# FudanCVL/SynFMC

Hardware: AMD Instinct MI355X
Metric: denoising steps/sec, 16x320x512 bf16 U-Net+CMC+OMC (higher is better)
Workload: dtype bf16; 1 GPU; 16x320x512 clip, CFG batch 2, full-width 3D U-Net (1.39B params, random init) + Camera Adapter (CMC) + Object Motion Control (OMC) features, DDIM step; configs/obj.yaml shapes; 1 clip per GPU; frames=16, height=320, width=512, hip_graph=True, fp8_temporal_attention=False, parallelism=dp1 (independent clips, no collective)

## Files before the change

include/fmc_hip.h:

```cpp
#ifndef FMC_HIP_H
#define FMC_HIP_H

#include <stdint.h>

#ifdef __cplusplus
extern "C" {
#endif

#define FMC_VERSION 100

enum { FMC_BF16 = 0, FMC_F32 = 1 };

enum {
    FMC_OK = 0,
    FMC_E_SHAPE = -1,
    FMC_E_DTYPE = -2,
    FMC_E_ALIGN = -3,
    FMC_E_LAUNCH = -4,
    FMC_E_NULL = -5
};

int fmc_version(void);
const char* fmc_last_error(void);

// ... 179 lines not shown
    int N, K;
    float alpha;
    int accumulate;
} fmc_wgrad_problem;
int64_t fmc_linear_wgrad_workspace_bytes(const fmc_wgrad_problem* problems, int n_problems);
int fmc_linear_wgrad_bf16(const fmc_wgrad_problem* problems, int n_problems, void* workspace, int64_t workspace_bytes, void* stream);

int fmc_temporal_block_bf16(const void* h, void* out, const float* ln_gamma, const float* ln_bpe, float ln_eps, const void* w_merge_tm,
                            const void* pose_term, float merge_scale, const void* w_qkv_packed, const void* w_out_tm, const void* b_out,
                            float* ln_stats, float ln_stats_eps, int n_clips, int frames, int hw, int channels, int heads, float scale,
                            void* stream);
int fmc_xattn_block640_bf16(const void* h, void* out, const float* ln_gamma, const float* ln_bpe, float ln_eps, const void* w_q_packed,
                            const void* kvfrag, const void* w_out_frag, const void* b_out, int n_images, int hw, int n_keys, int images_per_text,
                            float scale, void* stream);
int fmc_xattn_pack_kv(const void* kv, void* out, int batch, int S, int64_t ld_batch, void* stream);
int fmc_xattn_block320_bf16(const void* h, void* out, const float* ln_gamma, const float* ln_bpe, float ln_eps, const void* w_q_packed,
                            const void* kvfrag, const void* w_out_tm, const void* b_out, float* ln_stats, float ln_stats_eps, int n_images, int hw,
                            int n_keys, int images_per_text, float scale, void* stream);
int fmc_xattn_pack_kv40(const void* kv, void* out, int batch, int S, int64_t ld_batch, void* stream);
int fmc_geglu640_ln_bf16(const void* h, void* out, const float* ln_gamma, const float* ln_beta, float ln_eps, const void* w_packed, const void* bias,
                         int64_t M, int cff, int out_blocked, void* stream);
int fmc_geglu320_ln_bf16(const void* h, void* out, const float* ln_gamma, const float* ln_beta, float ln_eps, const void* w_packed, const void* bias,
                         int64_t M, int cff, int out_blocked, void* stream);
int fmc_temporal_block_set_debug(void* buf);

enum { FMC_OPTIM_ZERO_GRAD = 1 };
typedef struct fmc_optim_tensor {
    float* p;
    float* g;
    float* m;
    float* v;
    uint16_t* shadow_bf16;
    float* shadow_f32;
    float* step;
    int64_t n;
    int32_t clip_group;
    int32_t hyper_group;
    int32_t flags;
    int32_t reserved;
} fmc_optim_tensor;
typedef struct fmc_optim_chunk {
    int32_t tensor;
    int32_t chunk;
} fmc_optim_chunk;
int fmc_optim_chunk_elems(void);
int64_t fmc_optim_workspace_bytes(int n_tensors, int n_chunks, int n_clip_groups);
int fmc_optim_check_tables(const fmc_optim_tensor* h_tensors, int n_tensors, const fmc_optim_chunk* h_chunks, int n_chunks, int n_hyper,
                           int n_clip_groups);
int fmc_optim_grad_norm(const fmc_optim_tensor* tensors, int n_tensors, const fmc_optim_chunk* chunks, int n_chunks, const float* hyper,
                        int n_hyper, int n_clip_groups, void* workspace, int64_t workspace_bytes, void* stream);
int fmc_optim_adamw_step(const fmc_optim_tensor* tensors, int n_tensors, const fmc_optim_chunk* chunks, int n_chunks, const float* hyper,
                         int n_hyper, int n_clip_groups, void* workspace, int64_t workspace_bytes, void* stream);

#ifdef __cplusplus
}
#endif
#endif
```

synfmc_amd/_lib.py:

```python
from __future__ import annotations

import ctypes
import os
from ctypes import c_char_p, c_float, c_int, c_int64, c_void_p

_HERE = os.path.dirname(os.path.abspath(__file__))
LIB_PATH = os.environ.get("FMC_HIP_LIB") or os.path.join(_HERE, "lib", "libfmc_hip.so")

FMC_BF16, FMC_F32 = 0, 1

_ERRORS = {-1: ValueError, -2: TypeError, -3: ValueError, -4: RuntimeError, -5: ValueError}

SIGNATURES = {
    "fmc_version": (c_int, []),
    "fmc_last_error": (c_char_p, []),
    "fmc_groupnorm_workspace_bytes": (c_int64, [c_int, c_int, c_int]),
    "fmc_groupnorm_silu_fwd": (c_int, [c_void_p, c_void_p, c_void_p, c_void_p, c_void_p, c_void_p, c_int, c_int, c_int,
                                       c_int, c_float, c_int, c_int, c_void_p, c_int, c_void_p]),
    "fmc_groupnorm_silu_bwd": (c_int, [c_void_p, c_void_p, c_void_p, c_void_p, c_void_p, c_void_p, c_void_p, c_int,
                                       c_int, c_int, c_int, c_int, c_int, c_void_p]),
    "fmc_layernorm_add_fwd": (c_int, [c_void_p, c_void_p, c_void_p, c_void_p, c_void_p, c_void_p, c_void_p, c_int64, c_int, c_float, c_int,
                                      c_int, c_int, c_void_p]),
    "fmc_layernorm_fwd": (c_int, [c_void_p, c_void_p, c_void_p, c_void_p, c_void_p, c_int64, c_int, c_float, c_int,
                                  c_int, c_int, c_void_p]),
# ... 61 lines not shown
    "fmc_attention_fwd": (c_int, [c_void_p, c_void_p, c_void_p, c_void_p, c_void_p, c_int, c_int, c_int, c_int, c_int, c_int64, c_int64, c_int64, c_int64,
                                  c_int64, c_int64, c_float, c_int, c_int, c_void_p]),
    "fmc_vendor_init": (c_int, []),
    "fmc_vendor_destroy": (c_int, []),
    "fmc_vendor_version": (c_int, []),
    "fmc_vendor_workspace_bytes": (c_int64, []),
    "fmc_linear4_bf16": (c_int, [c_void_p, c_void_p, c_void_p, c_void_p, c_void_p, c_void_p, c_int64, c_int, c_int, c_int64, c_int64, c_int64, c_float, c_void_p]),
    "fmc_groupnorm_coef": (c_int, [c_void_p, c_int, c_void_p, c_void_p, c_void_p, c_void_p, c_int, c_int, c_int, c_int, c_float, c_void_p]),
    "fmc_groupnorm_apply_fwd": (c_int, [c_void_p, c_void_p, c_void_p, c_void_p, c_void_p, c_void_p, c_int, c_int, c_int, c_int, c_int,
                                        c_float, c_int, c_int, c_void_p]),
    "fmc_split_bf16x3": (c_int, [c_void_p, c_void_p, c_int64, c_int, c_int64, c_int64, c_int, c_int, c_int, c_void_p]),
    "fmc_linear_x3_f32": (c_int, [c_void_p, c_void_p, c_void_p, c_void_p, c_void_p, c_int64, c_int, c_int, c_int64,
                                  c_int64, c_int64, c_float, c_int, c_int, c_int, c_void_p, c_int64, c_void_p, c_void_p]),
    "fmc_conv3x3_x3_f32": (c_int, [c_void_p, c_void_p, c_void_p, c_void_p, c_void_p, c_void_p, c_int, c_int, c_int,
                                   c_int, c_int, c_int64, c_int, c_int, c_int, c_int, c_void_p, c_int64, c_void_p]),
    "fmc_layernorm_bwd": (c_int, [c_void_p, c_void_p, c_void_p, c_void_p, c_void_p, c_void_p, c_int64, c_int, c_float,
                                  c_int, c_void_p]),
    "fmc_layernorm_bwd_add": (c_int, [c_void_p, c_void_p, c_void_p, c_void_p, c_void_p, c_void_p, c_void_p, c_int64, c_int, c_float,
                                      c_int, c_void_p]),
    "fmc_groupnorm_silu_bwd_add": (c_int, [c_void_p, c_void_p, c_void_p, c_void_p, c_void_p, c_void_p, c_void_p, c_int, c_int, c_int, c_int,
                                           c_int, c_void_p, c_int, c_void_p]),
    "fmc_groupnorm_silu_bwd_params_workspace_bytes": (c_int64, [c_int, c_int, c_int, c_int]),
    "fmc_groupnorm_silu_bwd_params": (c_int, [c_void_p] * 9 + [c_int, c_void_p] + [c_int] * 6 + [c_void_p]),
    "fmc_column_sum_workspace_bytes": (c_int64, [c_int64, c_int]),
    "fmc_column_sum": (c_int, [c_void_p, c_void_p, c_int64, c_int, c_int64, c_float, c_int, c_void_p, c_int, c_void_p]),
    "fmc_geglu_bwd": (c_int, [c_void_p, c_void_p, c_void_p, c_int64, c_int, c_int, c_void_p]),
    "fmc_spatial_attn_bwd": (c_int, [c_void_p] * 10 + [c_int] * 5 + [c_int64] * 10 + [c_int, c_float, c_int, c_void_p]),
    "fmc_temporal_attn_bwd": (c_int, [c_void_p] * 7 + [c_int] * 5 + [c_int64] * 9 + [c_float, c_int, c_void_p]),
    "fmc_fp8_scales_roll": (c_int, [c_void_p, c_void_p, c_void_p, c_float, c_void_p]),
    "fmc_linear_fp8_qkv": (c_int, [c_void_p, c_void_p, c_void_p, c_int64, c_int, c_int, c_int64, c_void_p, c_void_p, c_void_p]),
    "fmc_temporal_attn_fp8_fwd": (c_int, [c_void_p] * 5 + [c_int] * 5 + [c_int64] * 6 + [c_float, c_void_p]),
    "fmc_temporal_attn_fp8_bwd": (c_int, [c_void_p] * 8 + [c_int] * 5 + [c_int64] * 9 + [c_float, c_void_p]),
    "fmc_nhwc_to_cmajor_padded": (c_int, [c_void_p, c_void_p, c_int, c_int, c_int, c_int, c_int64, c_int, c_int, c_void_p]),
    "fmc_linear_wgrad_workspace_bytes": (c_int64, [c_void_p, c_int]),
    "fmc_linear_wgrad_bf16": (c_int, [c_void_p, c_int, c_void_p, c_int64, c_void_p]),
    "fmc_optim_chunk_elems": (c_int, []),
    "fmc_optim_workspace_bytes": (c_int64, [c_int, c_int, c_int]),
    "fmc_optim_check_tables": (c_int, [c_void_p, c_int, c_void_p, c_int, c_int, c_int]),
    "fmc_optim_grad_norm": (c_int, [c_void_p, c_int, c_void_p, c_int, c_void_p, c_int, c_int, c_void_p, c_int64, c_void_p]),
    "fmc_optim_adamw_step": (c_int, [c_void_p, c_int, c_void_p, c_int, c_void_p, c_int, c_int, c_void_p, c_int64, c_void_p]),
    "fmc_temporal_block_bf16": (c_int, [c_void_p, c_void_p, c_void_p, c_void_p, c_float, c_void_p, c_void_p, c_float, c_void_p, c_void_p, c_void_p,
                                        c_void_p, c_float, c_int, c_int, c_int, c_int, c_int, c_float, c_void_p]),
    "fmc_temporal_block_set_debug": (c_int, [c_void_p]),
    "fmc_xattn_block640_bf16": (c_int, [c_void_p, c_void_p, c_void_p, c_void_p, c_float, c_void_p, c_void_p, c_void_p, c_void_p, c_int, c_int, c_int, c_int,
                                        c_float, c_void_p]),
    "fmc_xattn_pack_kv": (c_int, [c_void_p, c_void_p, c_int, c_int, c_int64, c_void_p]),
    "fmc_geglu320_ln_bf16": (c_int, [c_void_p, c_void_p, c_void_p, c_void_p, c_float, c_void_p, c_void_p, c_int64, c_int, c_int, c_void_p]),
    "fmc_geglu640_ln_bf16": (c_int, [c_void_p, c_void_p, c_void_p, c_void_p, c_float, c_void_p, c_void_p, c_int64, c_int, c_int, c_void_p]),
    "fmc_xattn_pack_kv40": (c_int, [c_void_p, c_void_p, c_int, c_int, c_int64, c_void_p]),
    "fmc_xattn_block320_bf16": (c_int, [c_void_p, c_void_p, c_void_p, c_void_p, c_float, c_void_p, c_void_p, c_void_p, c_void_p, c_void_p, c_float,
                                        c_int, c_int, c_int, c_int, c_float, c_void_p]),
    "fmc_conv3x3_bf16": (c_int, [c_void_p, c_void_p, c_void_p, c_void_p, c_void_p, c_void_p, c_int, c_int, c_int,
                                 c_int, c_int, c_int64, c_int, c_int, c_int, c_int, c_void_p, c_int64, c_void_p]),
}

_lib = None


class FmcLibraryMissing(ImportError):
    pass


def load() -> ctypes.CDLL:
    global _lib
    if _lib is not None:
        return _lib
    if not os.path.isfile(LIB_PATH):
        raise FmcLibraryMissing(
            f"{LIB_PATH} not found: build it with `make -C synfmc_amd/csrc` (hipcc --offload-arch=gfx950). "
            "There is no fallback path.")
    import torch
    lib = ctypes.CDLL(LIB_PATH)
    for name, (res, args) in SIGNATURES.items():
        fn = getattr(lib, name)
        fn.restype, fn.argtypes = res, args
    _lib = lib
    return lib


def check(rc: int, what: str) -> None:
    if rc != 0:
        msg = load().fmc_last_error()
        raise _ERRORS.get(rc, RuntimeError)(f"{what} failed ({rc}): {msg.decode() if msg else '?'}")
```

synfmc_amd/csrc/norm_kernels.hip:

```cpp
#include "common.h"

namespace {

constexpr int GN_MAX_SPLIT = 64;
constexpr int GN_MAX_G = 64;

struct GnGeom {
    int tpr;
    int rpi;
    int block;
    int split;
    int rows_per_split;
};

constexpr int GN_U = 4;

GnGeom gn_geom(int HW, int C) {
    GnGeom g;
    g.tpr = C / 8;
    g.rpi = 512 / g.tpr;
    if (g.rpi < 1) g.rpi = 1;
    if (g.rpi > HW) g.rpi = HW;
    g.block = g.tpr * g.rpi;
    int rows_target = 8 * g.rpi;
// ... 303 lines not shown
    int n, slab;
    if (xcd_order) {
        const int id = blockIdx.x, xcd = id & 7, within = id >> 3;
        n = (within / nslab) * 8 + xcd;
        slab = within % nslab;
    } else {
        n = blockIdx.y;
        slab = blockIdx.x;
    }
    const int CPS = CS / 8, cpg = C / G, GPB = CS / cpg;
    const int ch = tid % CPS, pl = tid / CPS;
    const int c0 = slab * CS + ch * 8;
    int xs = C;
    const T* xb = x + (size_t)n * HW * C + c0;
    if (x2) {
        xs = c0 < C1 ? C1 : C - C1;
        xb = c0 < C1 ? x + (size_t)n * HW * C1 + c0 : x2 + (size_t)n * HW * (C - C1) + (c0 - C1);
    }
    typename Vec8<T>::raw_t v[MAXCH];
    float gm[8], bt[8];
    Vec8<float>::load(gamma + c0, gm);
    Vec8<float>::load(beta + c0, bt);
    float s1[8], s2[8];
#pragma unroll
    for (int i = 0; i < 8; ++i) s1[i] = s2[i] = 0.f;
#pragma unroll
    for (int j = 0; j < MAXCH; ++j) {
        const int p = pl + PL * j;
        v[j] = Vec8<T>::load_raw(xb + (size_t)(p < HW ? p : HW - 1) * xs);
    }
#pragma unroll
    for (int j = 0; j < MAXCH; ++j) {
        const float m = (pl + PL * j) < HW ? 1.f : 0.f;
        float f[8];
        Vec8<T>::unpack(v[j], f);
#pragma unroll
        for (int i = 0; i < 8; ++i) { const float t = f[i] * m; s1[i] += t; s2[i] += t * f[i]; }
    }
    float* l1 = smem;
    float* l2 = smem + (size_t)PL * CS;
#pragma unroll
    for (int i = 0; i < 8; ++i) {
        l1[pl * CS + ch * 8 + i] = s1[i];
        l2[pl * CS + ch * 8 + i] = s2[i];
    }
    __syncthreads();
    for (int c = tid; c < CS; c += blockDim.x) {
        float a = 0.f, b = 0.f;
        for (int r = 0; r < PL; ++r) { a += l1[r * CS + c]; b += l2[r * CS + c]; }
        l1[c] = a;
        l2[c] = b;
    }
    __syncthreads();
    if (tid < GPB) {
        double a = 0.0, b = 0.0;
        for (int c = tid * cpg; c < (tid + 1) * cpg; ++c) { a += (double)l1[c]; b += (double)l2[c]; }
        const double cnt = (double)HW * cpg, mean = a / cnt;
        double var = b / cnt - mean * mean;
        if (var < 0.0) var = 0.0;
        const float rstd = (float)(1.0 / sqrt(var + (double)eps));
        sh_mean[tid] = (float)mean;
        sh_rstd[tid] = rstd;
        const int g = slab * GPB + tid;
        stats[((size_t)n * G + g) * 2] = (float)mean;
        stats[((size_t)n * G + g) * 2 + 1] = rstd;
    }
    __syncthreads();
    float aco[8], bco[8];
#pragma unroll
    for (int i = 0; i < 8; ++i) {
        const int gl = (ch * 8 + i) / cpg;
        aco[i] = sh_rstd[gl] * gm[i];
        bco[i] = bt[i] - sh_mean[gl] * aco[i];
    }
    T* yb = y + (size_t)n * HW * C + c0;
    if constexpr (sizeof(T) == 2) {
#pragma unroll
        for (int j = 0; j < MAXCH; ++j) asm volatile("" : "+v"(v[j]));
    }
#pragma unroll
    for (int j = 0; j < MAXCH; ++j) {
        const int p = pl + PL * j;
        if (p < HW) {
            float o[8], f[8];
            Vec8<T>::unpack(v[j], f);
#pragma unroll
            for (int i = 0; i < 8; ++i) {
                const float z = f[i] * aco[i] + bco[i];
                o[i] = act ? silu_f(z) : z;
            }
            Vec8<T>::store(yb + (size_t)p * C, o);
        }
    }
}

struct Gn1Geom { int CS, PL, block, chunks; };
static bool gn1_geom(int HW, int C, int G, Gn1Geom& out) {
    const int cpg = C / G;
    int best = 0, best_score = -1;
    for (int gpb = 1; gpb <= G; ++gpb) {
        if (G % gpb || gpb > GN_MAX_G) continue;
        const int cs = gpb * cpg;
        if (cs % 8) continue;
        const int cps = cs / 8;
        if (cps > 256) break;
        const int pl = 256 / cps < HW ? 256 / cps : HW;
        const int chunks = (HW + pl - 1) / pl;
        if (chunks > GN1_MAXCH) continue;
        if ((size_t)2 * pl * cs * sizeof(float) > 60 * 1024) continue;
        const int run = cs * 2 < 160 ? cs * 2 : 160;
        const int score = run * 1024 - chunks * 8 - gpb;
        if (score > best_score) { best_score = score; best = gpb; }
    }
    if (!best) return false;
    out.CS = best * cpg;
    const int cps = out.CS / 8;
// ... 892 lines not shown
```

synfmc_amd/hip_ops.py:

```python
from __future__ import annotations

import atexit
import math
import os
from typing import Optional, Tuple

import torch

from . import _lib
from ._lib import FMC_BF16, FMC_F32
from .derived import derived_on_owner

_DT = {torch.bfloat16: FMC_BF16, torch.float32: FMC_F32}


def _dt(t: torch.Tensor) -> int:
    try:
        return _DT[t.dtype]
    except KeyError:
        raise TypeError(f"fmc kernels take bf16 or fp32 activations, got {t.dtype}") from None


def _dev(*ts: torch.Tensor) -> None:
    for t in ts:
# ... 1781 lines not shown

def conv3x3_upfold_arm(n: int, hs: int, ws: int, cin: int, cout: int) -> Optional[str]:
    if not (UPS_FOLD and CONV_HALO) or ws < UPS_FOLD_MIN_WS:
        return None
    L = _lib.load()
    if (L.fmc_conv3x3_halo_fold_supported(n, hs, ws, cin, cout)
            and n * L.fmc_conv3x3_halo_tiles_per_image(hs, ws) * 4 * (cout // 160) >= CONV_HALO_MIN_TILES):
        return "halo"
    if not CONV_HALO4:
        return None
    wide = UPS_FOLD_WIDE and bool(L.fmc_conv3x3_halo4_fold_supported(n, hs, ws, cin, cout, 1))
    if (L.fmc_conv3x3_halo4_fold_supported(n, hs, ws, cin, cout, int(wide))
            and 4 * L.fmc_conv3x3_halo4_tiles(n, hs, ws, cout, int(wide)) >= CONV_HALO_MIN_TILES):
        return "halo4w" if wide else "halo4"
    return None


def _w_upfold_packed(weight_cl: torch.Tensor, tile_channels: int) -> torch.Tensor:
    return _w_packed(weight_cl, "upfold%d" % tile_channels, 16, "fmc_conv3x3_upfold_pack_weight", tile_channels)


def conv3x3_upfold(x_nhwc: torch.Tensor, weight_cl: torch.Tensor, bias=None, emit_gn: bool = False, arm: Optional[str] = None):
    _dev(x_nhwc, weight_cl, bias)
    n, hs, ws, cin = x_nhwc.shape
    cout = weight_cl.shape[0]
    assert x_nhwc.is_contiguous() and x_nhwc.dtype == torch.bfloat16 and weight_cl.dtype == torch.bfloat16 and weight_cl.shape[1] == cin
    assert not (torch.is_grad_enabled() and (x_nhwc.requires_grad or weight_cl.requires_grad)), "conv3x3_upfold: inference only"
    if arm is None:
        arm = conv3x3_upfold_arm(n, hs, ws, cin, cout)
    if arm not in ("halo", "halo4", "halo4w"):
        raise ValueError(f"conv3x3_upfold: no phase-mode launch for n={n} {hs}x{ws} {cin}->{cout} (arm {arm})")
    L = _lib.load()
    out = torch.empty(n, 2 * hs, 2 * ws, cout, dtype=x_nhwc.dtype, device=x_nhwc.device)
    shape, flops = (n, 2 * hs, 2 * ws, cin, cout, True), 2.0 * n * 4 * hs * ws * cout * 9 * cin
    conv_halo_calls["upfold"] = conv_halo_calls.get("upfold", 0) + 1
    if arm == "halo":
        wp = _w_upfold_packed(weight_cl, 160)
        part = torch.empty(n, 4 * L.fmc_conv3x3_halo_tiles_per_image(hs, ws), 32, 2, dtype=torch.float32, device=x_nhwc.device) if emit_gn else None
        conv_halo_calls["conv"] += 1
        if call_log is not None:
            call_log.append(("conv_halo", shape, flops))
        _lib.check(L.fmc_conv3x3_halo_fold_bf16(x_nhwc.data_ptr(), wp.data_ptr(), _p(bias), out.data_ptr(), n, hs, ws, cin, cout, _p(part), _stream()),
                   "fmc_conv3x3_halo_fold_bf16")
    else:
        wide = arm == "halo4w"
        wp = _w_upfold_packed(weight_cl, 160 if wide else 80)
        part = torch.empty(n, 4 * L.fmc_conv3x3_halo4_row_blocks_per_image(hs, ws), 32, 2, dtype=torch.float32, device=x_nhwc.device) if emit_gn else None
        conv_halo_calls["conv4"] = conv_halo_calls.get("conv4", 0) + 1
        if call_log is not None:
            call_log.append(("conv_halo4", shape, flops))
        _lib.check(L.fmc_conv3x3_halo4_fold_bf16(x_nhwc.data_ptr(), wp.data_ptr(), _p(bias), out.data_ptr(), n, hs, ws, cin, cout, _p(part), int(wide),
                                                 _stream()), "fmc_conv3x3_halo4_fold_bf16")
    return (out, part) if emit_gn else out


F32_GEMM = os.environ.get("FMC_F32_GEMM", "1") != "0"
f32_gemm_calls = {"linear": 0, "geglu": 0, "conv3x3": 0}


def split_bf16x3(src: torch.Tensor, role: int, dst: Optional[torch.Tensor] = None, col0: int = 0, K: Optional[int] = None) -> torch.Tensor:
    _dev(src)
    assert src.dtype == torch.float32
    C = src.shape[-1]
    rows, ld = _rows2d(src)
    K = C if K is None else K
    if dst is None:
        dst = torch.empty(rows, 3 * K, dtype=torch.bfloat16, device=src.device)
    assert dst.shape == (rows, 3 * K) and dst.is_contiguous()
    _lib.check(_lib.load().fmc_split_bf16x3(src.data_ptr(), dst.data_ptr(), rows, C, ld, 3 * K, col0, K, role, _stream()),
               "fmc_split_bf16x3")
    return dst


def _split_weight_cached(weight: torch.Tensor, rows: int, C: int) -> torch.Tensor:
    def build():
        w2 = weight.detach()
        w2 = w2.contiguous(memory_format=torch.channels_last).permute(0, 2, 3, 1).reshape(rows, C) if weight.ndim == 4 else w2.reshape(rows, C)
        return split_bf16x3(w2.contiguous(), 1)
    return derived_on_owner(weight, "_fmc_w3", (rows, C), build)


def _f32_arm(key_bf16, tile: int) -> int:
    if tile:
        return tile
    return _f32_arm_of(_choice.get(key_bf16, 0))


def _f32_arm_of(use: int) -> int:
    if ARM_160 <= use < ARM_160 + 5 or ARM_160B <= use < ARM_160B + 5 or use == ARM_256:
        return ARM_160
    if use >= 384:
        use -= 384
    elif use >= 256:
        use -= 256
    elif use >= 128:
        use -= 128
    if 16 <= use < 128:
        use &= 15
    return use if 1 <= use <= 14 else 0


def linear_f32(x: torch.Tensor, weight: torch.Tensor, bias=None, residual=None, alpha: float = 1.0, geglu: bool = False,
               tile: int = 0, split_k: int = 1, x2=None, residual2=None) -> torch.Tensor:
    tile, split_k = _decode_arm(tile, split_k)
    if split_k < 1:
        split_k = 1
# ... 855 lines not shown
```

synfmc_amd/models/unet.py:

```python
from __future__ import annotations

import inspect
import json
import os
from typing import Any, Dict, List, Optional, Tuple, Union

import torch
from torch import nn
import torch.nn.functional as F

from ..derived import derived
from .attention_processor import (AttnProcessor, LORAPoseAdaptorAttnProcessor, LoRAAttnProcessor,
                                  PoseAdaptorAttnProcessor)
from .layers import GroupNorm, TimestepEmbedding, Timesteps
from .resnet import InflatedConv3d, _frames_back, _frames_first
from .unet_blocks import (CrossAttnDownBlock3D, CrossAttnUpBlock3D, DownBlock3D, UNetMidBlock3DCrossAttn, UpBlock3D,
                          get_down_block, get_up_block)

CustomizedAttnProcessor = AttnProcessor
CustomizedLoRAAttnProcessor = LoRAAttnProcessor
WEIGHTS_NAME = "diffusion_pytorch_model.bin"


class UNet3DConditionOutput:
    def __init__(self, sample: torch.Tensor):
        self.sample = sample

    def __getitem__(self, i):
        return (self.sample,)[i]


class FrozenConfig(dict):

    def __getattr__(self, k):
        try:
            return self[k]
        except KeyError:
            raise AttributeError(k) from None


def _capture_config(obj, local_vars, cls):
    sig = inspect.signature(cls.__init__)
    cfg = {k: local_vars[k] for k in sig.parameters if k not in ("self", "kwargs") and k in local_vars}
    prev = dict(getattr(obj, "config", {}))
    prev.update(cfg)
    obj.config = FrozenConfig(prev)


class UNet3DConditionModel(nn.Module):
    _supports_gradient_checkpointing = True

    def __init__(self, sample_size: Optional[int] = None, in_channels: int = 4, out_channels: int = 4,
                 center_input_sample: bool = False, flip_sin_to_cos: bool = True, freq_shift: int = 0,
                 down_block_types: Tuple[str] = ("CrossAttnDownBlock3D", "CrossAttnDownBlock3D",
                                                 "CrossAttnDownBlock3D", "DownBlock3D"),
                 mid_block_type: str = "UNetMidBlock3DCrossAttn",
                 up_block_types: Tuple[str] = ("UpBlock3D", "CrossAttnUpBlock3D", "CrossAttnUpBlock3D",
                                               "CrossAttnUpBlock3D"),
                 only_cross_attention: Union[bool, Tuple[bool]] = False,
                 block_out_channels: Tuple[int] = (320, 640, 1280, 1280), layers_per_block: int = 2,
                 downsample_padding: int = 1, mid_block_scale_factor: float = 1, act_fn: str = "silu",
                 norm_num_groups: int = 32, norm_eps: float = 1e-5, cross_attention_dim: int = 1280,
                 attention_head_dim: Union[int, Tuple[int]] = 8, dual_cross_attention: bool = False,
                 use_linear_projection: bool = False, class_embed_type: Optional[str] = None,
                 addition_embed_type: Optional[str] = None, num_class_embeds: Optional[int] = None,
                 upcast_attention: bool = False, resnet_time_scale_shift: str = "default",
                 use_motion_module=False, motion_module_resolutions=(1, 2, 4, 8), motion_module_mid_block=False,
# ... 245 lines not shown
        return hit[1]

    def prepare_text_conditioning(self, encoder_hidden_states, cross_attention_kwargs=None) -> int:
        from .layers import BasicTransformerBlock
        n = 0
        with torch.no_grad():
            text = self._text_in_model_dtype(encoder_hidden_states)
            for m in self.modules():
                if isinstance(m, BasicTransformerBlock):
                    n += bool(m.prepare_text(text, cross_attention_kwargs))
        return n

    def invalidate_text_conditioning(self) -> None:
        self.__dict__.pop("_text_cast", None)
        for m in self.modules():
            if m.__dict__.get("_text_kv") is not None:
                m.__dict__.pop("_text_kv", None)

    def _resnets_with_temb(self):
        rs = getattr(self, "_temb_resnets", None)
        if rs is None:
            from .layers import ResnetBlock2D
            rs = [m for m in self.modules() if isinstance(m, ResnetBlock2D) and m.time_emb_proj is not None]
            object.__setattr__(self, "_temb_resnets", rs)
        return rs

    def _project_time_embedding(self, emb, frames):
        rs = self._resnets_with_temb()
        if torch.is_grad_enabled() or not rs or not emb.is_cuda or emb.dtype != torch.bfloat16 \
                or os.environ.get("FMC_NO_TEMB_BATCH"):
            return
        w, b = derived(self, "_temb_cat", [r.time_emb_proj.weight for r in rs],
                       lambda: (torch.cat([r.time_emb_proj.weight.detach() for r in rs], 0).to(emb.dtype),
                                torch.cat([r.time_emb_proj.bias.detach() for r in rs], 0).to(emb.dtype)))
        t_all = F.linear(F.silu(emb), w, b)
        from .. import hip_ops as K
        K._log_call("vendor", (emb.shape[0], w.shape[0], w.shape[1], True, False), 2.0 * emb.shape[0] * w.numel())
        off = 0
        for r in rs:
            co = r.time_emb_proj.weight.shape[0]
            r._t_pre = (t_all[:, off:off + co], frames)
            off += co

    def _run_blocks(self, sample, emb, encoder_hidden_states, attention_mask, cross_attention_kwargs,
                    pose_embedding_features, traj_features, use_pose, return_dict, upsample_size,
                    forward_upsample_size, cfg_shared_input: bool = False):
        if sample.dtype != self.dtype:
            sample = sample.to(self.dtype)
        encoder_hidden_states = self._text_in_model_dtype(encoder_hidden_states)
        shared = (cfg_shared_input and not torch.is_grad_enabled() and sample.shape[0] % 2 == 0
                  and len(self.down_blocks[0].resnets) > 0)
        if shared:
            sample = sample[: sample.shape[0] // 2]
        sample = self.conv_in(sample)
        if shared:
            self.down_blocks[0].__dict__["_cfg_half_input"] = True
            down_block_res_samples = (torch.cat([sample, sample], dim=0),)
        else:
            down_block_res_samples = (sample,)
        for i, downsample_block in enumerate(self.down_blocks):
            pf = pose_embedding_features[i] if use_pose else None
            mkw = {"pose_feature": pf} if use_pose else {}
            if getattr(downsample_block, "has_cross_attention", False):
                ckw = cross_attention_kwargs
                if use_pose:
                    ckw = {"pose_feature": pf}
                    if traj_features is not None or self._pass_traj_none:
                        ckw["traj_features"] = traj_features
                sample, res_samples = downsample_block(
                    hidden_states=sample, temb=emb, encoder_hidden_states=encoder_hidden_states,
                    attention_mask=attention_mask, cross_attention_kwargs=ckw if ckw is not None else {},
                    motion_cross_attention_kwargs=mkw)
            else:
                sample, res_samples = downsample_block(hidden_states=sample, temb=emb,
                                                       cross_attention_kwargs={"pose_feature": pf} if use_pose else None,
                                                       motion_cross_attention_kwargs=mkw)
            down_block_res_samples += res_samples
        mid_kw = {"pose_feature": pose_embedding_features[-1]} if use_pose else cross_attention_kwargs
        sample = self.mid_block(sample, emb, encoder_hidden_states=encoder_hidden_states,
                                attention_mask=attention_mask, cross_attention_kwargs=mid_kw,
                                motion_cross_attention_kwargs=mid_kw if use_pose else None)
        dec_pose = use_pose and getattr(self, "decoder_add_posecond", True)
        for i, upsample_block in enumerate(self.up_blocks):
            is_final_block = i == len(self.up_blocks) - 1
            n_res = len(upsample_block.resnets)
            res_samples = down_block_res_samples[-n_res:]
            down_block_res_samples = down_block_res_samples[:-n_res]
            if not is_final_block and forward_upsample_size:
                upsample_size = down_block_res_samples[-1].shape[-2:]
            pf = pose_embedding_features[-(i + 1)] if dec_pose else None
            mkw = {"pose_feature": pf} if dec_pose else {}
            ckw = {"pose_feature": pf} if dec_pose else cross_attention_kwargs
            if getattr(upsample_block, "has_cross_attention", False):
                sample = upsample_block(hidden_states=sample, temb=emb, res_hidden_states_tuple=res_samples,
                                        encoder_hidden_states=encoder_hidden_states, upsample_size=upsample_size,
                                        attention_mask=attention_mask, cross_attention_kwargs=ckw,
                                        motion_cross_attention_kwargs=mkw)
            else:
                sample = upsample_block(hidden_states=sample, temb=emb, res_hidden_states_tuple=res_samples,
                                        upsample_size=upsample_size, cross_attention_kwargs=ckw,
                                        motion_cross_attention_kwargs=mkw)
        x4, b, f = _frames_first(sample)
        x4 = self.conv_norm_out(x4, act=True)
        sample = self.conv_out(_frames_back(x4, b, f))
        if not return_dict:
            return (sample,)
        return UNet3DConditionOutput(sample=sample)

    _pass_traj_none = False
    _accepts_cfg_shared_input = True

    def forward(self, sample, timestep, encoder_hidden_states, class_labels=None, attention_mask=None,
                cross_attention_kwargs=None, return_dict: bool = True, down_block_additional_residuals=None,
                mid_block_additional_residual=None, motion_module_alphas=1.0, debug: bool = False,
                cfg_shared_input: bool = False):
        if down_block_additional_residuals is not None or mid_block_additional_residual is not None:
            raise NotImplementedError("ControlNet residuals are unused by FMC")
        return self._run(sample, timestep, encoder_hidden_states, attention_mask, cross_attention_kwargs, None, None,
                         False, return_dict, cfg_shared_input)


class UNet3DConditionModelPoseCond(UNet3DConditionModel):

    def __init__(self, decoder_add_posecond=True, **kwargs):
        super().__init__(**kwargs)
        self.decoder_add_posecond = decoder_add_posecond
        self.config = FrozenConfig({**self.config, "decoder_add_posecond": decoder_add_posecond})

    def set_all_attn_processor(self, add_spatial=False, spatial_attn_names="attn1", add_temporal=False,
                               add_spatial_lora=True, add_motion_lora=False, temporal_attn_names="0",
                               pose_feature_dimensions=[320, 640, 1280, 1280], lora_kwargs={}, motion_lora_kwargs={},
                               **attention_processor_kwargs):
        lora_kwargs, motion_lora_kwargs = dict(lora_kwargs), dict(motion_lora_kwargs)
        lora_rank = lora_kwargs.pop("lora_rank")
        motion_lora_rank = motion_lora_kwargs.pop("lora_rank")
        pfd = list(pose_feature_dimensions)

        def build(names, temporal, add_pose, add_lora, rank_cfg, selected, extra):
            chosen, procs = selected.split(","), {}
            for name in names:
                attn_name = name.split(".")[-2]
                hidden, idx, is_up = self._block_width(name)
                if temporal:
                    cross = None
                elif add_pose:
                    cross = None if attn_name == "attn1" else self.config.cross_attention_dim
                else:
                    cross = None if name.endswith("attn1.processor") else self.config.cross_attention_dim
                pose = add_pose and attn_name in chosen
                if pose and temporal and is_up:
                    pose = self.decoder_add_posecond
                pdim = (list(reversed(pfd))[idx] if is_up else pfd[idx]) if pose else None
                rank = (rank_cfg if rank_cfg > 16 else hidden // rank_cfg) if add_lora else None
                if pose and add_lora:
                    procs[name] = LORAPoseAdaptorAttnProcessor(hidden_size=hidden, pose_feature_dim=pdim,
                                                               cross_attention_dim=cross, rank=rank,
                                                               **attention_processor_kwargs, **extra)
# ... 40 lines not shown
```

Measured before the change: 39.94 steps/s.

## Add direct edge kernels for U-Net conv_in and fused GroupNorm-SiLU-conv_out

Adds two specialised HIP kernels for the U-Net edges. The first is a conv_in kernel for small Cin (4 or 8) that uses MFMA with a pre-packed filter held in LDS, and it can write the CFG-duplicated output directly. The second fuses GroupNorm apply, SiLU and the tiny-Cout conv_out, writing the result straight into the frames-back layout. Together they remove a torch.cat copy, the separate normalised activation tensor and the layout permutes, in exchange for more custom code paths with their own shape guards.

Result: no change. 40.14 steps/s (median of 6 runs) (+0.5%).

```diff
diff --git a/include/fmc_hip.h b/include/fmc_hip.h
--- a/include/fmc_hip.h
+++ b/include/fmc_hip.h
@@ -255,6 +255,15 @@
 int fmc_optim_adamw_step(const fmc_optim_tensor* tensors, int n_tensors, const fmc_optim_chunk* chunks, int n_chunks, const float* hyper,
                          int n_hyper, int n_clip_groups, void* workspace, int64_t workspace_bytes, void* stream);
 
+int fmc_conv3x3_in_supported(int n_img, int H, int W, int Cin, int Cout);
+int64_t fmc_conv3x3_in_packed_bytes(int Cin, int Cout);
+int fmc_conv3x3_in_pack_weight(const void* w, void* dst, int Cin, int Cout, void* stream);
+int fmc_conv3x3_in_bf16(const void* x, const void* w_packed, const void* bias, void* out, int n_img, int H, int W, int Cin, int Cout, int dup,
+                        void* stream);
+int fmc_conv3x3_norm_out_supported(int n_img, int H, int W, int C, int Cout, int frames);
+int fmc_conv3x3_norm_out_bf16(const void* x, const float* coef, const void* w, const void* bias, void* out, int n_img, int H, int W, int C, int Cout,
+                              int frames, void* stream);
+
 #ifdef __cplusplus
 }
 #endif
diff --git a/synfmc_amd/_lib.py b/synfmc_amd/_lib.py
--- a/synfmc_amd/_lib.py
+++ b/synfmc_amd/_lib.py
@@ -137,6 +137,12 @@
                                         c_int, c_int, c_int, c_int, c_float, c_void_p]),
     "fmc_conv3x3_bf16": (c_int, [c_void_p, c_void_p, c_void_p, c_void_p, c_void_p, c_void_p, c_int, c_int, c_int,
                                  c_int, c_int, c_int64, c_int, c_int, c_int, c_int, c_void_p, c_int64, c_void_p]),
+    "fmc_conv3x3_in_supported": (c_int, [c_int, c_int, c_int, c_int, c_int]),
+    "fmc_conv3x3_in_packed_bytes": (c_int64, [c_int, c_int]),
+    "fmc_conv3x3_in_pack_weight": (c_int, [c_void_p, c_void_p, c_int, c_int, c_void_p]),
+    "fmc_conv3x3_in_bf16": (c_int, [c_void_p, c_void_p, c_void_p, c_void_p, c_int, c_int, c_int, c_int, c_int, c_int, c_void_p]),
+    "fmc_conv3x3_norm_out_supported": (c_int, [c_int, c_int, c_int, c_int, c_int, c_int]),
+    "fmc_conv3x3_norm_out_bf16": (c_int, [c_void_p, c_void_p, c_void_p, c_void_p, c_void_p, c_int, c_int, c_int, c_int, c_int, c_int, c_void_p]),
 }
 
 _lib = None
diff --git a/synfmc_amd/csrc/conv_edge.hip b/synfmc_amd/csrc/conv_edge.hip
--- /dev/null
+++ b/synfmc_amd/csrc/conv_edge.hip
@@ -0,0 +1,306 @@
+#include "common.h"
+
+namespace {
+
+__device__ __forceinline__ float silu_f(float z) { return z * __builtin_amdgcn_rcpf(1.f + __expf(-z)); }
+
+union Frag { bf16x8 v; u32x4 u; u32x2 h[2]; bf16_t s[8]; };
+
+__device__ __forceinline__ f32x4 mfma(const bf16x8& a, const bf16x8& b, const f32x4& c) {
+    return __builtin_amdgcn_mfma_f32_16x16x32_bf16(a, b, c, 0, 0, 0);
+}
+
+__device__ __forceinline__ int tap_pixel(int tap, int y, int x, int H, int W, bool& ok) {
+    const int t = tap < 9 ? tap : 8;
+    const int yy = y + t / 3 - 1, xx = x + t % 3 - 1;
+    ok = tap < 9 && yy >= 0 && yy < H && xx >= 0 && xx < W;
+    return min(max(yy, 0), H - 1) * W + min(max(xx, 0), W - 1);
+}
+
+constexpr int IN_BAND = 64, IN_THREADS = 256, IN_MAX_KSTEPS = 3;
+
+struct InParams {
+    const bf16_t* x; const bf16_t* w; const bf16_t* bias; bf16_t* out;
+    int n_img, H, W, cin, cout, dup;
+    int kp, cout32;
+};
+
+__host__ __device__ inline int in_kp(int cin) { return (9 * cin + 31) / 32 * 32; }
+__host__ __device__ inline int in_row(int kp) { return kp + 8; }
+
+__global__ __launch_bounds__(256) void conv_in_pack_kernel(const bf16_t* __restrict__ w, bf16_t* __restrict__ dst, int cin, int cout) {
+    const int kp = in_kp(cin), rs = in_row(kp), cout32 = (cout + 31) / 32 * 32;
+    for (int i = blockIdx.x * blockDim.x + threadIdx.x; i < cout32 * rs; i += gridDim.x * blockDim.x) {
+        const int row = i / rs, k = i - row * rs;
+        const int m = row & 15, j = (row >> 4) & 1;
+        const int co = (row & ~31) + 8 * (m >> 2) + 4 * j + (m & 3);
+        dst[i] = (co < cout && k < 9 * cin) ? w[(size_t)co * 9 * cin + k] : (bf16_t)0;
+    }
+}
+
+__device__ __forceinline__ bf16x8 in_operand(const bf16_t* __restrict__ img, int y, int x, int H, int W, int cin, int k0) {
+    Frag f;
+    bool ok;
+    if (cin == 8) {
+        const int p = tap_pixel(k0 >> 3, y, x, H, W, ok);
+        const u32x4 v = *reinterpret_cast<const u32x4*>(img + (size_t)p * 8);
+        f.u = ok ? v : u32x4{0u, 0u, 0u, 0u};
+    } else if (cin == 4) {
+#pragma unroll
+        for (int t = 0; t < 2; ++t) {
+            const int p = tap_pixel((k0 >> 2) + t, y, x, H, W, ok);
+            const u32x2 v = *reinterpret_cast<const u32x2*>(img + (size_t)p * 4);
+            f.h[t] = ok ? v : u32x2{0u, 0u};
+        }
+    } else {
+#pragma unroll
+        for (int e = 0; e < 8; ++e) {
+            const int k = k0 + e, tap = k / cin, ci = k - tap * cin;
+            const int p = tap_pixel(tap, y, x, H, W, ok);
+            const bf16_t v = img[(size_t)p * cin + ci];
+            f.s[e] = ok ? v : (bf16_t)0;
+        }
+    }
+    return f.v;
+}
+
+__global__ __launch_bounds__(IN_THREADS) void conv_in_kernel(const InParams P) {
+    extern __shared__ __attribute__((aligned(16))) unsigned char smem[];
+    const int rs = in_row(P.kp);
+    bf16_t* sw = reinterpret_cast<bf16_t*>(smem);
+    float* sb = reinterpret_cast<float*>(smem + (size_t)P.cout32 * rs * 2);
+    const int tid = threadIdx.x, lane = tid & 63, wave = tid >> 6;
+    {
+        const u32x4* src = reinterpret_cast<const u32x4*>(P.w);
+        u32x4* dst = reinterpret_cast<u32x4*>(smem);
+        const int pieces = P.cout32 * rs / 8;
+        for (int i = tid; i < pieces; i += IN_THREADS) dst[i] = src[i];
+        for (int c = tid; c < P.cout32; c += IN_THREADS) sb[c] = (P.bias && c < P.cout) ? bf2f(P.bias[c]) : 0.f;
+    }
+    __syncthreads();
+    const int HW = P.H * P.W, n = blockIdx.y;
+    const int p0 = blockIdx.x * IN_BAND, p1 = min(p0 + IN_BAND, HW);
+    const bf16_t* img = P.x + (size_t)n * HW * P.cin;
+    const int m = lane & 15, q = lane >> 4;
+    const int nks = P.kp >> 5;
+    for (int pb = p0 + wave * 16; pb < p1; pb += (IN_THREADS / 64) * 16) {
+        const int p = pb + m;
+        const bool valid = p < p1;
+        const int pc = valid ? p : p1 - 1;
+        const int y = pc / P.W, x = pc - y * P.W;
+        bf16x8 b[IN_MAX_KSTEPS];
+#pragma unroll
+        for (int s = 0; s < IN_MAX_KSTEPS; ++s)
+            if (s < nks) b[s] = in_operand(img, y, x, P.H, P.W, P.cin, 32 * s + 8 * q);
+        bf16_t* o0 = P.out + ((size_t)n * HW + pc) * P.cout;
+        bf16_t* o1 = o0 + (size_t)P.n_img * HW * P.cout;
+        for (int c0 = 0; c0 < P.cout32; c0 += 32) {
+            f32x4 acc0 = {0.f, 0.f, 0.f, 0.f}, acc1 = {0.f, 0.f, 0.f, 0.f};
+            const bf16_t* a = sw + (size_t)(c0 + m) * rs + 8 * q;
+#pragma unroll
+            for (int s = 0; s < IN_MAX_KSTEPS; ++s)
+                if (s < nks) {
+                    acc0 = mfma(*reinterpret_cast<const bf16x8*>(a + 32 * s), b[s], acc0);
+                    acc1 = mfma(*reinterpret_cast<const bf16x8*>(a + 16 * rs + 32 * s), b[s], acc1);
+                }
+            const int c = c0 + 8 * q;
+            if (valid && c < P.cout) {
+                float v[8];
+#pragma unroll
+                for (int i = 0; i < 4; ++i) { v[i] = acc0[i] + sb[c + i]; v[4 + i] = acc1[i] + sb[c + 4 + i]; }
+                Vec8<bf16_t>::store(o0 + c, v);
+                if (P.dup) Vec8<bf16_t>::store(o1 + c, v);
+            }
+        }
+    }
+}
+
+constexpr int OUT_TH = 8, OUT_TW = 16, OUT_THREADS = 256, OUT_WAVES = OUT_THREADS / 64;
+constexpr int OUT_HW = OUT_TW + 2, OUT_HALO = (OUT_TH + 2) * OUT_HW;
+constexpr int OUT_PS = 72;
+constexpr int OUT_MAX_COUT = 8;
+constexpr int OUT_PIECES = (OUT_HALO * 8 + OUT_THREADS - 1) / OUT_THREADS;
+constexpr int OUT_WPIECES = (OUT_MAX_COUT * 9 * 8 + OUT_THREADS - 1) / OUT_THREADS;
+static_assert(OUT_TW == 16 && OUT_TH == 2 * OUT_WAVES && OUT_THREADS % 8 == 0, "a wave owns two tile rows of 16 pixels; a thread stages one channel group");
+
+struct OutParams {
+    const bf16_t* x; const float* coef; const bf16_t* w; const bf16_t* bias; bf16_t* out;
+    int n_img, H, W, C, cout, frames, tiles_x, tiles, xcd_order;
+};
+
+struct OutStage {
+    u32x4 raw[OUT_PIECES], wraw[OUT_WPIECES];
+    float sc[8], sh[8];
+    bool inside[OUT_PIECES];
+};
+
+__device__ __forceinline__ void out_request(OutStage& S, const OutParams& P, const bf16_t* __restrict__ img, const float* __restrict__ coef, int y0, int x0,
+                                            int cc, int tid) {
+    const int cbase = cc * 64 + (tid & 7) * 8;
+    const bool chan_ok = cbase < P.C;
+#pragma unroll
+    for (int i = 0; i < OUT_PIECES; ++i) {
+        const int hp = (tid + i * OUT_THREADS) >> 3;
+        const int hr = hp / OUT_HW, yy = y0 - 1 + hr, xx = x0 - 1 + (hp - hr * OUT_HW);
+        S.inside[i] = chan_ok && hp < OUT_HALO && yy >= 0 && yy < P.H && xx >= 0 && xx < P.W;
+        const size_t off = S.inside[i] ? ((size_t)yy * P.W + xx) * P.C + cbase : 0;
+        S.raw[i] = *reinterpret_cast<const u32x4*>(img + off);
+    }
+    const f32x4* cp = reinterpret_cast<const f32x4*>(coef + (chan_ok ? cbase : 0) * 2);
+#pragma unroll
+    for (int i = 0; i < 4; ++i) {
+        const f32x4 v = cp[i];
+        S.sc[2 * i] = v[0]; S.sh[2 * i] = v[1]; S.sc[2 * i + 1] = v[2]; S.sh[2 * i + 1] = v[3];
+    }
+    const int wrows = P.cout * 9;
+#pragma unroll
+    for (int i = 0; i < OUT_WPIECES; ++i) {
+        const int row = (tid + i * OUT_THREADS) >> 3;
+        const bool ok = chan_ok && row < wrows;
+        const u32x4 v = *reinterpret_cast<const u32x4*>(P.w + (ok ? (size_t)row * P.C + cbase : 0));
+        S.wraw[i] = ok ? v : u32x4{0u, 0u, 0u, 0u};
+    }
+}
+
+__global__ __launch_bounds__(OUT_THREADS) void conv_norm_out_kernel(const OutParams P) {
+    __shared__ __attribute__((aligned(16))) bf16_t s_x[OUT_HALO * OUT_PS];
+    __shared__ __attribute__((aligned(16))) bf16_t s_w[OUT_MAX_COUT * 9 * OUT_PS];
+    const int tid = threadIdx.x, lane = tid & 63, wave = tid >> 6;
+    int n = blockIdx.y, tile = blockIdx.x;
+    if (P.xcd_order) {
+        const int within = blockIdx.x >> 3;
+        n = (within / P.tiles) * 8 + (blockIdx.x & 7);
+        tile = within % P.tiles;
+    }
+    const int ty = tile / P.tiles_x, tx = tile - ty * P.tiles_x;
+    const int y0 = ty * OUT_TH, x0 = tx * OUT_TW;
+    const int m = lane & 15, q = lane >> 4;
+    const int pg = tid & 7;
+    const bf16_t* img = P.x + (size_t)n * P.H * P.W * P.C;
+    const float* coef = P.coef + (size_t)n * P.C * 2;
+    f32x4 acc[2] = {{0.f, 0.f, 0.f, 0.f}, {0.f, 0.f, 0.f, 0.f}};
+    const int nchunk = (P.C + 63) / 64;
+    OutStage S;
+    out_request(S, P, img, coef, y0, x0, 0, tid);
+    for (int cc = 0; cc < nchunk; ++cc) {
+        __syncthreads();
+#pragma unroll
+        for (int i = 0; i < OUT_PIECES; ++i) {
+            const int hp = (tid + i * OUT_THREADS) >> 3;
+            if (hp < OUT_HALO) {
+                float v[8];
+                Vec8<bf16_t>::unpack(S.raw[i], v);
+#pragma unroll
+                for (int k = 0; k < 8; ++k) {
+                    const float z = v[k] * S.sc[k] + S.sh[k];
+                    v[k] = S.inside[i] ? silu_f(z) : 0.f;
+                }
+                Vec8<bf16_t>::store(s_x + hp * OUT_PS + pg * 8, v);
+            }
+        }
+#pragma unroll
+        for (int i = 0; i < OUT_WPIECES; ++i) {
+            const int row = (tid + i * OUT_THREADS) >> 3;
+            if (row < OUT_MAX_COUT * 9) *reinterpret_cast<u32x4*>(s_w + row * OUT_PS + pg * 8) = S.wraw[i];
+        }
+        __syncthreads();
+        if (cc + 1 < nchunk) out_request(S, P, img, coef, y0, x0, cc + 1, tid);
+        const bf16_t* arow = s_w + (m < P.cout ? m : 0) * 9 * OUT_PS + 8 * q;
+#pragma unroll
+        for (int tap = 0; tap < 9; ++tap) {
+            Frag a0, a1;
+            a0.v = *reinterpret_cast<const bf16x8*>(arow + tap * OUT_PS);
+            a1.v = *reinterpret_cast<const bf16x8*>(arow + tap * OUT_PS + 32);
+            if (m >= P.cout) { a0.u = u32x4{0u, 0u, 0u, 0u}; a1.u = u32x4{0u, 0u, 0u, 0u}; }
+#pragma unroll
+            for (int g = 0; g < 2; ++g) {
+                const bf16_t* bp = s_x + ((wave + OUT_WAVES * g + tap / 3) * OUT_HW + m + tap % 3) * OUT_PS + 8 * q;
+                acc[g] = mfma(a0.v, *reinterpret_cast<const bf16x8*>(bp), acc[g]);
+                acc[g] = mfma(a1.v, *reinterpret_cast<const bf16x8*>(bp + 32), acc[g]);
+            }
+        }
+    }
+    const int b = n / P.frames, f = n - b * P.frames;
+    const size_t HW = (size_t)P.H * P.W;
+#pragma unroll
+    for (int g = 0; g < 2; ++g) {
+        const int y = y0 + wave + OUT_WAVES * g, x = x0 + m;
+        if (y < P.H && x < P.W)
+#pragma unroll
+            for (int i = 0; i < 4; ++i) {
+                const int co = 4 * q + i;
+                if (co < P.cout)
+                    P.out[(((size_t)b * P.cout + co) * P.frames + f) * HW + (size_t)y * P.W + x] = f2bf(acc[g][i] + (P.bias ? bf2f(P.bias[co]) : 0.f));
+            }
+    }
+}
+
+}
+
+extern "C" int64_t fmc_conv3x3_in_packed_bytes(int Cin, int Cout) {
+    if (Cin < 1 || Cin > 8 || Cout < 16 || Cout % 16) return 0;
+    return (int64_t)((Cout + 31) / 32 * 32) * in_row(in_kp(Cin)) * 2;
+}
+
+static int64_t in_lds_bytes(int Cin, int Cout) { return fmc_conv3x3_in_packed_bytes(Cin, Cout) + (int64_t)((Cout + 31) / 32 * 32) * 4; }
+
+extern "C" int fmc_conv3x3_in_supported(int n_img, int H, int W, int Cin, int Cout) {
+    if (n_img < 1 || n_img > 65535 || H < 1 || W < 1 || Cin < 1 || Cin > 8 || Cout < 16 || Cout % 16) return 0;
+    if ((int64_t)H * W >= (1ll << 30)) return 0;
+    if (in_lds_bytes(Cin, Cout) > 128 * 1024) return 0;
+    return 1;
+}
+
+extern "C" int fmc_conv3x3_in_pack_weight(const void* w, void* dst, int Cin, int Cout, void* stream) {
+    if (!w || !dst) FMC_FAIL(FMC_E_NULL, "conv3x3_in_pack_weight: NULL pointer");
+    if (!fmc_conv3x3_in_packed_bytes(Cin, Cout)) FMC_FAIL(FMC_E_SHAPE, "conv3x3_in_pack_weight: needs Cin <= 8, Cout %% 16 == 0 (Cin=%d Cout=%d)", Cin, Cout);
+    if (!fmc_aligned16(dst)) FMC_FAIL(FMC_E_ALIGN, "conv3x3_in_pack_weight: dst must be 16-byte aligned");
+    const int total = (Cout + 31) / 32 * 32 * in_row(in_kp(Cin));
+    hipLaunchKernelGGL(conv_in_pack_kernel, dim3((unsigned)((total + 255) / 256)), dim3(256), 0, (hipStream_t)stream, (const bf16_t*)w, (bf16_t*)dst, Cin, Cout);
+    FMC_CHECK_LAUNCH("fmc_conv3x3_in_pack_weight");
+    return 0;
+}
+
+extern "C" int fmc_conv3x3_in_bf16(const void* x, const void* w_packed, const void* bias, void* out, int n_img, int H, int W, int Cin, int Cout, int dup,
+                                   void* stream) {
+    if (!x || !w_packed || !out) FMC_FAIL(FMC_E_NULL, "conv3x3_in: NULL x / w / out");
+    if (!fmc_conv3x3_in_supported(n_img, H, W, Cin, Cout))
+        FMC_FAIL(FMC_E_SHAPE, "conv3x3_in: needs Cin <= 8, Cout %% 16 == 0, the packed filter within 128 KiB (n=%d H=%d W=%d Cin=%d Cout=%d)", n_img, H, W, Cin, Cout);
+    if (!fmc_aligned16(x) || !fmc_aligned16(w_packed) || !fmc_aligned16(out) || (bias && (reinterpret_cast<uintptr_t>(bias) & 1)))
+        FMC_FAIL(FMC_E_ALIGN, "conv3x3_in: x / w / out must be 16-byte aligned");
+    InParams P;
+    P.x = (const bf16_t*)x; P.w = (const bf16_t*)w_packed; P.bias = (const bf16_t*)bias; P.out = (bf16_t*)out;
+    P.n_img = n_img; P.H = H; P.W = W; P.cin = Cin; P.cout = Cout; P.dup = dup ? 1 : 0;
+    P.kp = in_kp(Cin); P.cout32 = (Cout + 31) / 32 * 32;
+    const unsigned bands = (unsigned)(((int64_t)H * W + IN_BAND - 1) / IN_BAND);
+    fmc_launch<conv_in_kernel>(dim3(bands, (unsigned)n_img), dim3(IN_THREADS), (size_t)in_lds_bytes(Cin, Cout), (hipStream_t)stream, P);
+    FMC_CHECK_LAUNCH("fmc_conv3x3_in_bf16");
+    return 0;
+}
+
+extern "C" int fmc_conv3x3_norm_out_supported(int n_img, int H, int W, int C, int Cout, int frames) {
+    if (n_img < 1 || n_img > 65535 || H < 1 || W < 1 || C < 32 || C % 32 || Cout < 1 || Cout > OUT_MAX_COUT) return 0;
+    if (frames < 1 || n_img % frames) return 0;
+    if ((int64_t)H * W >= (1ll << 30) || (int64_t)((H + OUT_TH - 1) / OUT_TH) * ((W + OUT_TW - 1) / OUT_TW) >= (1ll << 31)) return 0;
+    return 1;
+}
+
+extern "C" int fmc_conv3x3_norm_out_bf16(const void* x, const float* coef, const void* w, const void* bias, void* out, int n_img, int H, int W, int C,
+                                         int Cout, int frames, void* stream) {
+    if (!x || !coef || !w || !out) FMC_FAIL(FMC_E_NULL, "conv3x3_norm_out: NULL x / coef / w / out");
+    if (!fmc_conv3x3_norm_out_supported(n_img, H, W, C, Cout, frames))
+        FMC_FAIL(FMC_E_SHAPE, "conv3x3_norm_out: needs C %% 32 == 0, Cout <= 8, n_img %% frames == 0 (n=%d H=%d W=%d C=%d Cout=%d frames=%d)", n_img, H, W, C,
+                 Cout, frames);
+    if (!fmc_aligned16(x) || !fmc_aligned16(coef) || !fmc_aligned16(w) || (reinterpret_cast<uintptr_t>(out) & 1) || (bias && (reinterpret_cast<uintptr_t>(bias) & 1)))
+        FMC_FAIL(FMC_E_ALIGN, "conv3x3_norm_out: x / coef / w must be 16-byte aligned");
+    OutParams P;
+    P.x = (const bf16_t*)x; P.coef = coef; P.w = (const bf16_t*)w; P.bias = (const bf16_t*)bias; P.out = (bf16_t*)out;
+    P.n_img = n_img; P.H = H; P.W = W; P.C = C; P.cout = Cout; P.frames = frames;
+    P.tiles_x = (W + OUT_TW - 1) / OUT_TW;
+    P.tiles = P.tiles_x * ((H + OUT_TH - 1) / OUT_TH);
+    P.xcd_order = n_img % 8 == 0 && (int64_t)P.tiles * n_img < (1ll << 31);
+    const dim3 grid = P.xcd_order ? dim3((unsigned)(P.tiles * n_img)) : dim3((unsigned)P.tiles, (unsigned)n_img);
+    fmc_launch<conv_norm_out_kernel>(grid, dim3(OUT_THREADS), 0, (hipStream_t)stream, P);
+    FMC_CHECK_LAUNCH("fmc_conv3x3_norm_out_bf16");
+    return 0;
+}
diff --git a/synfmc_amd/csrc/norm_kernels.hip b/synfmc_amd/csrc/norm_kernels.hip
--- a/synfmc_amd/csrc/norm_kernels.hip
+++ b/synfmc_amd/csrc/norm_kernels.hip
@@ -379,16 +379,16 @@
         l2[c] = b;
     }
     __syncthreads();
-    if (tid < GPB) {
+    for (int gl = tid; gl < GPB; gl += blockDim.x) {
         double a = 0.0, b = 0.0;
-        for (int c = tid * cpg; c < (tid + 1) * cpg; ++c) { a += (double)l1[c]; b += (double)l2[c]; }
+        for (int c = gl * cpg; c < (gl + 1) * cpg; ++c) { a += (double)l1[c]; b += (double)l2[c]; }
         const double cnt = (double)HW * cpg, mean = a / cnt;
         double var = b / cnt - mean * mean;
         if (var < 0.0) var = 0.0;
         const float rstd = (float)(1.0 / sqrt(var + (double)eps));
-        sh_mean[tid] = (float)mean;
-        sh_rstd[tid] = rstd;
-        const int g = slab * GPB + tid;
+        sh_mean[gl] = (float)mean;
+        sh_rstd[gl] = rstd;
+        const int g = slab * GPB + gl;
         stats[((size_t)n * G + g) * 2] = (float)mean;
         stats[((size_t)n * G + g) * 2 + 1] = rstd;
     }
diff --git a/synfmc_amd/hip_ops.py b/synfmc_amd/hip_ops.py
--- a/synfmc_amd/hip_ops.py
+++ b/synfmc_amd/hip_ops.py
@@ -1857,6 +1857,110 @@
         _lib.check(L.fmc_conv3x3_halo4_fold_bf16(x_nhwc.data_ptr(), wp.data_ptr(), _p(bias), out.data_ptr(), n, hs, ws, cin, cout, _p(part), int(wide),
                                                  _stream()), "fmc_conv3x3_halo4_fold_bf16")
     return (out, part) if emit_gn else out
+
+
+EDGE_DIRECT = os.environ.get("FMC_EDGE_DIRECT", "1") != "0"
+edge_direct_calls = {"conv_in": 0, "conv_norm_out": 0}
+
+
+def edge_in_packed_shape(cin: int, cout: int) -> Tuple[int, int]:
+    return (cout + 31) // 32 * 32, (9 * cin + 31) // 32 * 32 + 8
+
+
+def edge_in_row_channel(row: int) -> int:
+    m, j = row % 16, (row // 16) % 2
+    return row // 32 * 32 + 8 * (m // 4) + 4 * j + m % 4
+
+
+def edge_in_pack_reference(weight: torch.Tensor) -> torch.Tensor:
+    cout, cin = weight.shape[:2]
+    rows, rl = edge_in_packed_shape(cin, cout)
+    flat = weight.permute(0, 2, 3, 1).reshape(cout, 9 * cin)
+    out = torch.zeros(rows, rl, dtype=weight.dtype, device=weight.device)
+    chan = torch.tensor([edge_in_row_channel(r) for r in range(rows)], device=weight.device)
+    keep = chan < cout
+    out[keep, :9 * cin] = flat[chan[keep]]
+    return out
+
+
+def conv_norm_out_reference(x_nhwc: torch.Tensor, coef: torch.Tensor, weight: torch.Tensor, bias: Optional[torch.Tensor], frames: int = 1) -> torch.Tensor:
+    import torch.nn.functional as F
+    n, h, w, c = x_nhwc.shape
+    z = x_nhwc.float() * coef[:, None, None, :, 0].float() + coef[:, None, None, :, 1].float()
+    a = F.silu(z).bfloat16().float().permute(0, 3, 1, 2)
+    y = F.conv2d(a, weight.float(), None if bias is None else bias.float(), padding=1)
+    return y.view(n // frames, frames, weight.shape[0], h, w).permute(0, 2, 1, 3, 4).contiguous()
+
+
+def _edge_conv_ok(x_nchw: torch.Tensor, conv) -> bool:
+    w = conv.weight
+    return (EDGE_DIRECT and x_nchw.is_cuda and x_nchw.dtype == torch.bfloat16 and w.dtype == torch.bfloat16 and not torch.is_grad_enabled()
+            and (conv.bias is None or conv.bias.dtype == torch.bfloat16) and x_nchw.ndim == 4 and x_nchw.shape[1] == w.shape[1]
+            and tuple(w.shape[2:]) == (3, 3) and tuple(conv.stride) == (1, 1) and tuple(conv.padding) == (1, 1) and tuple(conv.dilation) == (1, 1)
+            and conv.groups == 1 and x_nchw.permute(0, 2, 3, 1).is_contiguous() and x_nchw.data_ptr() % 16 == 0)
+
+
+def conv_in_direct_ok(x_nchw: torch.Tensor, conv) -> bool:
+    if not _edge_conv_ok(x_nchw, conv):
+        return False
+    n, cin, h, w = x_nchw.shape
+    return bool(_lib.load().fmc_conv3x3_in_supported(n, h, w, cin, conv.weight.shape[0]))
+
+
+def _w_edge_in_packed(weight_cl: torch.Tensor) -> torch.Tensor:
+    def build():
+        cout, cin = weight_cl.shape[:2]
+        assert weight_cl.permute(0, 2, 3, 1).is_contiguous()
+        L = _lib.load()
+        out = torch.empty(L.fmc_conv3x3_in_packed_bytes(cin, cout) // 2, dtype=weight_cl.dtype, device=weight_cl.device)
+        _lib.check(L.fmc_conv3x3_in_pack_weight(weight_cl.data_ptr(), out.data_ptr(), cin, cout, _stream()), "fmc_conv3x3_in_pack_weight")
+        return out
+    return derived_on_owner(weight_cl, "_fmc_wtm", "edge_in", build)
+
+
+def conv_in_direct(x_nchw: torch.Tensor, weight_cl: torch.Tensor, bias: Optional[torch.Tensor] = None, dup: bool = False) -> torch.Tensor:
+    _dev(x_nchw, weight_cl, bias)
+    n, cin, h, w = x_nchw.shape
+    cout = weight_cl.shape[0]
+    wp = _w_edge_in_packed(weight_cl)
+    out = torch.empty(2 * n if dup else n, h, w, cout, dtype=x_nchw.dtype, device=x_nchw.device)
+    edge_direct_calls["conv_in"] += 1
+    dispatch_calls["conv3x3"]["own"] += 1
+    _log_call("conv_edge_in", (n, h, w, cin, cout, bool(dup)), 2.0 * n * h * w * cout * 9 * cin)
+    _lib.check(_lib.load().fmc_conv3x3_in_bf16(x_nchw.data_ptr(), wp.data_ptr(), _p(bias), out.data_ptr(), n, h, w, cin, cout, int(dup), _stream()),
+               "fmc_conv3x3_in_bf16")
+    return out.permute(0, 3, 1, 2)
+
+
+def conv_norm_out_direct_ok(x_nchw: torch.Tensor, norm, conv, frames: int = 1) -> bool:
+    if not _edge_conv_ok(x_nchw, conv) or norm.num_groups != 32 or norm.weight is None or norm.bias is None:
+        return False
+    n, c, h, w = x_nchw.shape
+    return bool(_lib.load().fmc_conv3x3_norm_out_supported(n, h, w, c, conv.weight.shape[0], frames))
+
+
+def conv_norm_out_direct(x_nchw: torch.Tensor, gamma: torch.Tensor, beta: torch.Tensor, eps: float, weight_cl: torch.Tensor,
+                         bias: Optional[torch.Tensor] = None, frames: int = 1, coef: Optional[torch.Tensor] = None) -> torch.Tensor:
+    _dev(x_nchw, gamma, beta, weight_cl, bias, coef)
+    n, c, h, w = x_nchw.shape
+    cout = weight_cl.shape[0]
+    assert weight_cl.permute(0, 2, 3, 1).is_contiguous() and n % frames == 0
+    if coef is None:
+        tag = getattr(x_nchw, "_fmc_gn", None)
+        if tag is not None and tag[1] == c and tag[0].shape[0] == n and tag[0].shape[2] == 32:
+            part = tag[0]
+            conv_halo_calls["stats_from_producer"] += 1
+        else:
+            part = groupnorm_partials(x_nchw.permute(0, 2, 3, 1).view(n, h * w, c), 32)
+        coef = groupnorm_coef(part, gamma, beta, h * w, c, 32, eps)
+    assert coef.shape == (n, c, 2) and coef.dtype == torch.float32 and coef.is_contiguous()
+    out = torch.empty(n // frames, cout, frames, h, w, dtype=x_nchw.dtype, device=x_nchw.device)
+    edge_direct_calls["conv_norm_out"] += 1
+    dispatch_calls["conv3x3"]["own"] += 1
+    _log_call("conv_edge_out", (n, h, w, c, cout), 2.0 * n * h * w * cout * 9 * c)
+    _lib.check(_lib.load().fmc_conv3x3_norm_out_bf16(x_nchw.data_ptr(), coef.data_ptr(), weight_cl.data_ptr(), _p(bias), out.data_ptr(), n, h, w, c, cout,
+                                                     frames, _stream()), "fmc_conv3x3_norm_out_bf16")
+    return out
 
 
 F32_GEMM = os.environ.get("FMC_F32_GEMM", "1") != "0"
diff --git a/synfmc_amd/models/unet.py b/synfmc_amd/models/unet.py
--- a/synfmc_amd/models/unet.py
+++ b/synfmc_amd/models/unet.py
@@ -12,7 +12,7 @@
 from ..derived import derived
 from .attention_processor import (AttnProcessor, LORAPoseAdaptorAttnProcessor, LoRAAttnProcessor,
                                   PoseAdaptorAttnProcessor)
-from .layers import GroupNorm, TimestepEmbedding, Timesteps
+from .layers import GroupNorm, TimestepEmbedding, Timesteps, f32_param
 from .resnet import InflatedConv3d, _frames_back, _frames_first
 from .unet_blocks import (CrossAttnDownBlock3D, CrossAttnUpBlock3D, DownBlock3D, UNetMidBlock3DCrossAttn, UpBlock3D,
                           get_down_block, get_up_block)
@@ -364,12 +364,18 @@
                   and len(self.down_blocks[0].resnets) > 0)
         if shared:
             sample = sample[: sample.shape[0] // 2]
-        sample = self.conv_in(sample)
+        from .. import hip_ops as K
+        x4 = None
+        if K.EDGE_DIRECT and sample.is_cuda and sample.dtype == torch.bfloat16 and not torch.is_grad_enabled():
+            x4, b, f = _frames_first(sample)
+        if x4 is not None and K.conv_in_direct_ok(x4, self.conv_in):
+            both = _frames_back(K.conv_in_direct(x4, self.conv_in._weight_cl(), self.conv_in.bias, dup=shared), 2 * b if shared else b, f)
+            sample, down_block_res_samples = (both[:b] if shared else both), (both,)
+        else:
+            sample = self.conv_in(sample)
+            down_block_res_samples = (torch.cat([sample, sample], dim=0),) if shared else (sample,)
         if shared:
             self.down_blocks[0].__dict__["_cfg_half_input"] = True
-            down_block_res_samples = (torch.cat([sample, sample], dim=0),)
-        else:
-            down_block_res_samples = (sample,)
         for i, downsample_block in enumerate(self.down_blocks):
             pf = pose_embedding_features[i] if use_pose else None
             mkw = {"pose_feature": pf} if use_pose else {}
@@ -413,8 +419,12 @@
                                         upsample_size=upsample_size, cross_attention_kwargs=ckw,
                                         motion_cross_attention_kwargs=mkw)
         x4, b, f = _frames_first(sample)
-        x4 = self.conv_norm_out(x4, act=True)
-        sample = self.conv_out(_frames_back(x4, b, f))
+        if K.conv_norm_out_direct_ok(x4, self.conv_norm_out, self.conv_out, f):
+            sample = K.conv_norm_out_direct(x4, f32_param(self.conv_norm_out, "weight"), f32_param(self.conv_norm_out, "bias"), self.conv_norm_out.eps,
+                                            self.conv_out._weight_cl(), self.conv_out.bias, f)
+        else:
+            x4 = self.conv_norm_out(x4, act=True)
+            sample = self.conv_out(_frames_back(x4, b, f))
         if not return_dict:
             return (sample,)
         return UNet3DConditionOutput(sample=sample)
```
